# simonamtoft/downsampled-diffusion

Measured on AMD Instinct MI355X. Metric: images/sec (T=1000 sampling), 256x256 dDDPM-x3, higher is better.
Workload: dtype f32

## Files before the change

### downsampled-diffusion_amd/csrc/attention.hip

```cpp
#include <cstdlib>

#include "cluster_sync.h"
#include "conv_common.h"

namespace ddk {

constexpr int DH = 32;

constexpr int PART = DH + DH + DH * DH;

__global__ __launch_bounds__(256) void linattn_context_kernel(const float* __restrict__ qkv, float* __restrict__ ctx,
                                                              float* __restrict__ part, int HW, int heads, int splits, int rows_per_split,
                                                              int kv_only) {
    __shared__ __attribute__((aligned(16))) float stage[4 * 32 * 33];
    float* kexp = stage;
    float* vs = stage + 64 * DH;
    __shared__ float smax[8 * DH];
    const int bh = blockIdx.x / splits, sp = blockIdx.x % splits;
    const int b = bh / heads, h = bh % heads;
    const int HC = heads * DH, RS = (kv_only ? 2 : 3) * HC;
    const float* base = qkv + (long long)b * HW * RS;
    const float* kp = base + (kv_only ? 0 : HC) + h * DH;
    const float* vp = kp + HC;
    const int tid = threadIdx.x;
// ... 650 lines not shown
constexpr int AS_REC = 1152;
constexpr int AS_CNT = 32;
constexpr int AS_RING = 4;

template <int ROWS>
struct AttnSplitGeom {
    static_assert(ROWS == 128 || ROWS == 32, "half of a 16x16 or of an 8x8 map");
    static constexpr int XP = ROWS / 8;
    static constexpr int NP = XP + 12;
    static constexpr int SLOT = (ROWS + 96) * 32;
    static constexpr int NB = ROWS == 128 ? 3 : 1;
    static constexpr int UNITS = ROWS == 128 ? 4 : 3;
    static constexpr int KPART = UNITS * NB * 16 * 64;
    static constexpr int SCR = KPART > 8 * 32 * 33 ? KPART : 8 * 32 * 33;
    static constexpr int RING_FL = AS_RING * SLOT;
    static_assert(SCR + 2 * ROWS * DH + ROWS * (DH + 1) <= RING_FL, "k, v, q of the half live behind the scratch area in the drained ring");
    static constexpr int TAIL = DH * (DH + 4) + 2 * ROWS + 16 * DH + 16 * DH + DH + 192 + AS_REC + 32;
    static constexpr int LDS_FL = RING_FL + TAIL;
};

struct AttnSplitParams {
    const float* x;
    const float* w;
    const float* c1;
    const float* c2;
    float eps;
    float* ctx;
    float* out;
    unsigned* cnt;
    float* rec;
    unsigned* fail;
    int C;
};

__device__ __forceinline__ void wait_vmcnt_le(int n) {
    if (n >= 8) wait_vmcnt<8>();
    else if (n >= 6) wait_vmcnt<6>();
    else if (n >= 4) wait_vmcnt<4>();
    else if (n >= 3) wait_vmcnt<3>();
    else if (n >= 2) wait_vmcnt<2>();
    else wait_vmcnt<0>();
}

template <int ROWS>
__global__ __launch_bounds__(512) void attn_split_kernel(const AttnSplitParams p) {
    using G = AttnSplitGeom<ROWS>;
    constexpr int HW = 2 * ROWS, HC = 4 * DH;
    extern __shared__ __attribute__((aligned(16))) float smem[];
    float* scr = smem;
    float* ks = smem + G::SCR;
    float* vs = ks + ROWS * DH;
    float* qs = vs + ROWS * DH;
    float* cs = smem + G::RING_FL;
    float* rowstat = cs + DH * (DH + 4);
    float* smax = rowstat + 2 * ROWS;
    float* dpart = smax + 16 * DH;
    float* mx = dpart + 16 * DH;
    float* cfold = mx + DH;
    float* own = cfold + 192;
    int* gave_up = reinterpret_cast<int*>(own + AS_REC);
    const int tid = threadIdx.x, lane = tid & 63;
    const int wid = __builtin_amdgcn_readfirstlane(tid >> 6);
    const int half = blockIdx.x, h = blockIdx.y, b = blockIdx.z;
    const int C = p.C, nch = C >> 5;
    const float* xb = p.x + ((long long)b * HW + half * ROWS) * C;
    const unsigned lds_base = (unsigned)(size_t)(__attribute__((address_space(3))) float*)smem;

    const int prow = lane >> 3, ppos = lane & 7;
    const int npw = (G::NP - wid + 7) >> 3;
    unsigned voff[4];
#pragma unroll
    for (int j = 0; j < 4; ++j) {
        const int pj = wid + 8 * j;
        const int r = 8 * (pj < G::XP ? pj : pj - G::XP) + prow;
        const int src = pj < G::XP ? r : (r >> 5) * HC + h * DH + (r & 31);
        voff[j] = (unsigned)((src * C + ((ppos ^ ((r >> 1) & 7)) << 2)) * 4);
    }
    auto issue = [&](int chunk) {
        const unsigned dst = lds_base + (unsigned)(((chunk & (AS_RING - 1)) * G::SLOT) * 4);
#pragma unroll
        for (int j = 0; j < 4; ++j) {
            const int pj = wid + 8 * j;
            if (pj < G::NP) lds_dma16_s(pj < G::XP ? xb : p.w, voff[j] + (unsigned)(chunk * 128), dst + (unsigned)(pj * 1024));
        }
    };
    for (int c = 0; c < AS_RING - 1 && c < nch; ++c) issue(c);
    if (tid < 192) {
        const int n = tid % 96;
        const int col = (n >> 5) * HC + h * DH + (n & 31);
        cfold[tid] = tid < 96 ? p.c1[col] : p.c2[col];
    }
    if (tid < 4 * ROWS) {
        const int row = tid >> 2, sub = tid & 3, n16 = C >> 4;
        const float4* rp = reinterpret_cast<const float4*>(xb + (long long)row * C);
        float4 v[16];
        float s = 0.f;
#pragma unroll
        for (int i = 0; i < 16; ++i)
            if (i < n16) {
                v[i] = rp[sub + 4 * i];
                s += (v[i].x + v[i].y) + (v[i].z + v[i].w);
            }
        s += __shfl_xor(s, 1, 64);
        s += __shfl_xor(s, 2, 64);
        const float inv_c = 1.0f / (float)C;
        const float mean = s * inv_c;
        float qq = 0.f;
#pragma unroll
        for (int i = 0; i < 16; ++i)
            if (i < n16) {
                const float a0 = v[i].x - mean, a1 = v[i].y - mean, a2 = v[i].z - mean, a3 = v[i].w - mean;
                qq += (a0 * a0 + a1 * a1) + (a2 * a2 + a3 * a3);
            }
        qq += __shfl_xor(qq, 1, 64);
        qq += __shfl_xor(qq, 2, 64);
        if (sub == 0) {
            const float r = 1.0f / (sqrtf(qq * inv_c) + p.eps);
            rowstat[2 * row] = r;
            rowstat[2 * row + 1] = r * mean;
        }
    }

    const int pl = lane & 31, hl = lane >> 5;
    const bool active = ROWS == 128 || wid < 6;
    const int kh = ROWS == 128 ? wid >> 2 : (wid >= 3 ? 1 : 0);
    const int unit = ROWS == 128 ? (wid & 3) : (wid >= 3 ? wid - 3 : wid);
    const int pb = ROWS == 128 ? unit : 0, blk0 = ROWS == 128 ? 0 : unit;
    f32x16 acc[G::NB];
#pragma unroll
    for (int i = 0; i < G::NB; ++i)
#pragma unroll
        for (int r = 0; r < 16; ++r) acc[i][r] = 0.f;
    const int fsw = (pl >> 1) & 7;
    for (int c = 0; c < nch; ++c) {
        const int later = nch - 1 - c < AS_RING - 2 ? nch - 1 - c : AS_RING - 2;
        wait_vmcnt_le(later * npw);
        asm volatile("s_waitcnt lgkmcnt(0)\n\ts_barrier" ::: "memory");
        if (c + AS_RING - 1 < nch) issue(c + AS_RING - 1);
        if (active) {
            const float* Xs = smem + (c & (AS_RING - 1)) * G::SLOT + pb * (32 * 32);
            const float* Ws = smem + (c & (AS_RING - 1)) * G::SLOT + ROWS * 32 + blk0 * (32 * 32);
#pragma unroll
            for (int q2 = 0; q2 < 2; ++q2) {
                const int off = pl * 32 + (((2 * (2 * kh + q2) + hl) ^ fsw) << 2);
                const float4 xv = *reinterpret_cast<const float4*>(Xs + off);
                float4 wv[G::NB];
#pragma unroll
                for (int i = 0; i < G::NB; ++i) wv[i] = *reinterpret_cast<const float4*>(Ws + i * (32 * 32) + off);
#pragma unroll
                for (int e = 0; e < 4; ++e) {
                    const float xe = e == 0 ? xv.x : e == 1 ? xv.y : e == 2 ? xv.z : xv.w;
#pragma unroll
                    for (int i = 0; i < G::NB; ++i)
                        acc[i] = __builtin_amdgcn_mfma_f32_32x32x2f32(e == 0 ? wv[i].x : e == 1 ? wv[i].y : e == 2 ? wv[i].z : wv[i].w, xe, acc[i], 0, 0, 0);
                }
            }
        }
    }
    __syncthreads();
    if (active && kh == 1) {
#pragma unroll
        for (int i = 0; i < G::NB; ++i)
#pragma unroll
            for (int r = 0; r < 16; ++r) scr[((unit * G::NB + i) * 16 + r) * 64 + lane] = acc[i][r];
    }
    __syncthreads();
    if (active && kh == 0) {
        const int n = pb * 32 + pl;
        const float r = rowstat[2 * n], rm = rowstat[2 * n + 1];
#pragma unroll
        for (int i = 0; i < G::NB; ++i) {
            const int blk = blk0 + i;
#pragma unroll
            for (int q = 0; q < 4; ++q) {
                const int d0 = 8 * q + 4 * hl;
                float o4[4];
#pragma unroll
                for (int e = 0; e < 4; ++e) {
                    const float a = acc[i][4 * q + e] + scr[((unit * G::NB + i) * 16 + 4 * q + e) * 64 + lane];
                    o4[e] = r * a - rm * cfold[blk * 32 + d0 + e] + cfold[96 + blk * 32 + d0 + e];
                }
                if (blk == 0) {
#pragma unroll
                    for (int e = 0; e < 4; ++e) qs[n * (DH + 1) + d0 + e] = o4[e];
                } else {
                    *reinterpret_cast<float4*>((blk == 1 ? ks : vs) + n * DH + d0) = make_float4(o4[0], o4[1], o4[2], o4[3]);
                }
            }
        }
    }
    __syncthreads();

    {
        const int d = tid & 31, ng = tid >> 5;
        float m = -INFINITY;
        for (int n = ng; n < ROWS; n += 16) m = fmaxf(m, ks[n * DH + d]);
        smax[ng * DH + d] = m;
        __syncthreads();
        if (tid < DH) {
            float mm = smax[tid];
#pragma unroll
            for (int j = 1; j < 16; ++j) mm = fmaxf(mm, smax[j * DH + tid]);
            mx[tid] = mm;
        }
        __syncthreads();
// ... 31 lines not shown
#pragma unroll
            for (int w = 1; w < 8; ++w) t += scr[(w * 32 + md) * 33 + me0 + e];
            own[2 * DH + md * DH + me0 + e] = t;
        }
        if (me0 == 0) { own[md] = mx[md]; own[DH + md] = den; }
    }
    __syncthreads();
    unsigned* cnt = p.cnt + (b * 4 + h) * AS_CNT;
    float* rec = p.rec + (long long)(b * 4 + h) * 2 * AS_REC;
    if (wid == 0) {
        unsigned* mine = reinterpret_cast<unsigned*>(rec + half * AS_REC);
#pragma unroll
        for (int i = 0; i < (2 * DH + DH * DH) / 64; ++i)
            __hip_atomic_store(mine + lane + 64 * i, __float_as_uint(own[lane + 64 * i]), __ATOMIC_RELAXED, __HIP_MEMORY_SCOPE_AGENT);
        asm volatile("s_waitcnt vmcnt(0)" ::: "memory");
        if (lane == 0) {
            __hip_atomic_fetch_add(cnt, 1u, __ATOMIC_RELAXED, __HIP_MEMORY_SCOPE_AGENT);
            *gave_up = cl_wait_ge<2>(cnt, 2u, p.fail) ? 1 : 0;
        }
    }
    __syncthreads();
    const bool poisoned = *gave_up != 0;
    if (tid < 256) {
        const unsigned* theirs = reinterpret_cast<const unsigned*>(rec + (half ^ 1) * AS_REC);
        const float tm = __uint_as_float(__hip_atomic_load(theirs + md, __ATOMIC_RELAXED, __HIP_MEMORY_SCOPE_AGENT));
        const float td = __uint_as_float(__hip_atomic_load(theirs + DH + md, __ATOMIC_RELAXED, __HIP_MEMORY_SCOPE_AGENT));
        float ta[4];
#pragma unroll
        for (int e = 0; e < 4; ++e)
            ta[e] = __uint_as_float(__hip_atomic_load(theirs + 2 * DH + md * DH + me0 + e, __ATOMIC_RELAXED, __HIP_MEMORY_SCOPE_AGENT));
        if (tid == 0) cl_depart(cnt, cnt + 1, 2u);
        const float om = own[md], od = own[DH + md];
        const float m0 = half ? tm : om, m1 = half ? om : tm;
        const float d0 = half ? td : od, d1 = half ? od : td;
        const float M = fmaxf(m0, m1);
// ... 9 lines not shown
            const float a0 = half ? ta[e] : oa, a1 = half ? oa : ta[e];
            float a = 0.f;
            a += a0 * w0;
            a += a1 * w1;
            c4[e] = a * inv;
            cs[md * (DH + 4) + me0 + e] = c4[e];
        }
        if (half == 0) *reinterpret_cast<float4*>(p.ctx + (((long long)b * 4 + h) * DH + md) * DH + me0) = make_float4(c4[0], c4[1], c4[2], c4[3]);
    }
    __syncthreads();
    if (wid < ROWS / 32) {
        const int n0 = wid * 32;
        f32x16 oacc;
#pragma unroll
        for (int r = 0; r < 16; ++r) oacc[r] = 0.f;
        const float* qp = qs + (n0 + pl) * (DH + 1) + hl;
        const float* cp = cs + hl * (DH + 4) + pl;
#pragma unroll
        for (int j = 0; j < DH / 2; ++j) oacc = __builtin_amdgcn_mfma_f32_32x32x2f32(qp[2 * j], cp[2 * j * (DH + 4)], oacc, 0, 0, 0);
        float* op = p.out + ((long long)b * HW + half * ROWS + n0) * HC + h * DH + pl;
#pragma unroll
        for (int r = 0; r < 16; ++r) op[((r & 3) + 8 * (r >> 2) + 4 * hl) * HC] = oacc[r];
    }
}

__global__ __launch_bounds__(256) void qkv_operand_pack_kernel(const float* __restrict__ lnw, float* __restrict__ wop, int heads, int cp,
                                                               long long total) {
    const int nch = cp >> 5, HC = heads * DH;
    for (long long idx = blockIdx.x * 256LL + threadIdx.x; idx < total; idx += (long long)gridDim.x * 256) {
        const int j = (int)(idx & 3), lane = (int)((idx >> 2) & 63), half = (int)((idx >> 8) & 1);
        long long r = idx >> 9;
        const int nb = (int)(r % 6); r /= 6;
        const int chunk = (int)(r % nch);
        const int head = (int)(r / nch);
        const int o = (nb >> 1) * HC + head * DH + (nb & 1) * 16 + (lane & 15);
        const int i = chunk * 32 + (lane >> 4) * 8 + half * 4 + j;
        wop[idx] = lnw[(long long)o * cp + i];
    }
// ... 178 lines not shown
            const int n = nq * 32 + tid;
            a1[(long long)b * FOLD_C + n] = u1;
            a2[(long long)b * FOLD_C + n] = u2 + (bout ? bout[n] : 0.f);
        }
    }
}

int linattn_small_qkv_init_device() {
    DDK_HIP(hipFuncSetAttribute(reinterpret_cast<const void*>(attn_kvctx_kernel), hipFuncAttributeMaxDynamicSharedMemorySize,
                                (int)(KC_LDS_FLOATS * sizeof(float))));
    DDK_HIP(hipFuncSetAttribute(reinterpret_cast<const void*>(attn_fold_kernel), hipFuncAttributeMaxDynamicSharedMemorySize,
                                (int)(FOLD_LDS_FLOATS * sizeof(float))));
    DDK_HIP(hipFuncSetAttribute(reinterpret_cast<const void*>(linattn_small_kernel<256>), hipFuncAttributeMaxDynamicSharedMemorySize, 160 * 1024));
    DDK_HIP(hipFuncSetAttribute(reinterpret_cast<const void*>(linattn_small_qkv_kernel<1>), hipFuncAttributeMaxDynamicSharedMemorySize, 160 * 1024));
    DDK_HIP(hipFuncSetAttribute(reinterpret_cast<const void*>(linattn_small_qkv_kernel<4>), hipFuncAttributeMaxDynamicSharedMemorySize, 160 * 1024));
    DDK_HIP(hipFuncSetAttribute(reinterpret_cast<const void*>(attn_split_kernel<128>), hipFuncAttributeMaxDynamicSharedMemorySize,
                                (int)(AttnSplitGeom<128>::LDS_FL * sizeof(float))));
    DDK_HIP(hipFuncSetAttribute(reinterpret_cast<const void*>(attn_split_kernel<32>), hipFuncAttributeMaxDynamicSharedMemorySize,
                                (int)(AttnSplitGeom<32>::LDS_FL * sizeof(float))));
    return DDK_OK;
}

int qkv_operand_pack(const float* lnw, float* wop, int heads, int cp, hipStream_t st) {
    DDK_REQUIRE(lnw && wop && heads > 0 && cp > 0 && cp % 32 == 0, "qkv_operand_pack: arguments");
    const long long total = (long long)3 * heads * DH * cp;
    const long long blocks = ceil_div(total, 256);
    hipLaunchKernelGGL(qkv_operand_pack_kernel, dim3((unsigned)(blocks < 2048 ? blocks : 2048)), dim3(256), 0, st, lnw, wop, heads, cp, total);
    return check_launch("qkv_operand_pack_kernel");
}

int linattn_small_qkv(const float* x, const float* wop, const float* c1, const float* c2, float ln_eps, float* ctx, float* out, int B, int HW,
                      int C, int heads, hipStream_t st) {
// ... 37 lines not shown
    hipLaunchKernelGGL(linattn_merge_kernel, dim3(B * 4), dim3(256), 0, st, static_cast<const float*>(workspace), ctx, s);
    return check_launch("linattn_merge_kernel");
}

constexpr int AS_CUS = 256;
bool attn_split_ok(int B, int HW, int C, int heads) {
    return B > 0 && (HW == 64 || HW == 256) && C >= 32 && C <= 256 && C % 32 == 0 && heads == 4 && 8 * (long long)B <= AS_CUS &&
           conv_wino_cluster_device_ok();
}
size_t attn_split_counter_words(int B) { return (size_t)B * 4 * AS_CNT; }
size_t attn_split_record_floats(int B) { return (size_t)B * 4 * 2 * AS_REC; }
size_t attn_split_workspace_bytes(int B) { return B > 0 ? (32 + attn_split_counter_words(B) + attn_split_record_floats(B)) * sizeof(float) : 0; }
unsigned attention_cluster_timeouts() { return cl_timeouts_read(); }

int attn_split(const float* x, const float* w, const float* c1, const float* c2, float ln_eps, float* ctx, float* out, int B, int HW, int C,
               unsigned* counters, float* records, unsigned* fail, hipStream_t st) {
    DDK_REQUIRE(x && w && c1 && c2 && ctx && out && counters && records, "attn_split: null pointer");
    DDK_REQUIRE(attn_split_ok(B, HW, C, 4), "attn_split: needs H*W of 64 or 256, C % 32 == 0, C <= 256, 4 heads, 8 * B <= the CU count of a whole MI355X");
    DDK_REQUIRE(aligned16(x) && aligned16(w) && aligned16(ctx) && aligned16(out) && aligned16(counters) && aligned16(records), "attn_split: alignment");
    DDK_TRY(ensure_device_init());
    const AttnSplitParams p{x, w, c1, c2, ln_eps, ctx, out, counters, records, fail, C};
    if (HW == 256)
        hipLaunchKernelGGL(attn_split_kernel<128>, dim3(2, 4, (unsigned)B), dim3(512), AttnSplitGeom<128>::LDS_FL * sizeof(float), st, p);
    else
        hipLaunchKernelGGL(attn_split_kernel<32>, dim3(2, 4, (unsigned)B), dim3(512), AttnSplitGeom<32>::LDS_FL * sizeof(float), st, p);
    return check_launch("attn_split_kernel");
}

bool attn_fold_ok(int C, int heads) { return C == FOLD_C && heads * DH == FOLD_C; }
size_t attn_fold_out_floats(int B) { return (size_t)B * (FOLD_C * FOLD_C + 2 * FOLD_C); }

int attn_fold(const float* ctx, const float* wqg, const float* c1q, const float* c2q, const float* wout, const float* bout, float* A,
              float* a1, float* a2, int B, int C, int heads, hipStream_t st) {
    DDK_REQUIRE(ctx && wqg && c1q && c2q && wout && A && a1 && a2 && B > 0, "attn_fold: arguments");
    DDK_REQUIRE(attn_fold_ok(C, heads), "attn_fold: C == 128 and heads * 32 == 128 only");
    DDK_REQUIRE(aligned16(ctx) && aligned16(wout) && aligned16(A), "attn_fold: alignment");
    DDK_TRY(ensure_device_init());
// ... 19 lines not shown
    return ddk::linattn_context(qkv, ctx, B, HW, heads, workspace, workspace_bytes, ddk::as_stream(s), false);
}
int ddk_linattn_context_kv(const float* kv, float* ctx, int B, int HW, int heads, void* workspace, size_t workspace_bytes, ddk_stream_t s) {
    return ddk::linattn_context(kv, ctx, B, HW, heads, workspace, workspace_bytes, ddk::as_stream(s), true);
}
size_t ddk_attention_kv_context_workspace_bytes(int B, int HW) { return ddk::attn_kvctx_workspace_bytes(B, HW); }
int ddk_attention_kv_context_ok(int B, int HW, int C, int heads) { return ddk::attn_kvctx_ok(B, HW, C, heads) ? 1 : 0; }
int ddk_attention_kv_context(const float* x, const float* w_kv, const float* c1, const float* c2, float ln_eps, float* ctx, int B, int HW,
                             void* workspace, size_t workspace_bytes, ddk_stream_t s) {
    return ddk::attn_kvctx(x, w_kv, c1, c2, ln_eps, ctx, B, HW, workspace, workspace_bytes, ddk::as_stream(s));
}
size_t ddk_attention_split_workspace_bytes(int B) { return ddk::attn_split_workspace_bytes(B); }
int ddk_attention_split_ok(int B, int HW, int C, int heads) { return ddk::attn_split_ok(B, HW, C, heads) ? 1 : 0; }
int ddk_attention_split_from_x(const float* x, const float* w_folded, const float* c1, const float* c2, float ln_eps, float* ctx, float* out,
                               int B, int HW, int C, int heads, void* workspace, size_t workspace_bytes, ddk_stream_t s) {
    using namespace ddk;
    DDK_REQUIRE(workspace && B > 0 && heads == 4, "attention_split_from_x: arguments (4 heads)");
    if (workspace_bytes < attn_split_workspace_bytes(B)) {
        set_error("attention_split_from_x: workspace too small (%zu < %zu)", workspace_bytes, attn_split_workspace_bytes(B));
        return DDK_ERR_WORKSPACE;
    }
    unsigned* words = static_cast<unsigned*>(workspace);
    return attn_split(x, w_folded, c1, c2, ln_eps, ctx, out, B, HW, C, words + 32, static_cast<float*>(workspace) + 32 + attn_split_counter_words(B),
                      words, as_stream(s));
}
int ddk_attention_fold(const float* ctx, const float* wqg, const float* c1q, const float* c2q, const float* wout, const float* bout, float* A,
                       float* a1, float* a2, int B, int C, int heads, ddk_stream_t s) {
    return ddk::attn_fold(ctx, wqg, c1q, c2q, wout, bout, A, a1, a2, B, C, heads, ddk::as_stream(s));
}
int ddk_linattn_fused_small(const float* qkv, float* ctx, float* out, int B, int HW, int heads, ddk_stream_t s) {
    return ddk::linattn_fused_small(qkv, ctx, out, B, HW, heads, ddk::as_stream(s));
}
int ddk_pack_qkv_operand(const float* folded_w, float* dst, int heads, int c_pad, ddk_stream_t s) {
    return ddk::qkv_operand_pack(folded_w, dst, heads, c_pad, ddk::as_stream(s));
}
int ddk_linattn_small_from_x(const float* x, const float* w_operand, const float* c1, const float* c2, float ln_eps, float* ctx, float* out,
                             int B, int HW, int C, int heads, ddk_stream_t s) {
    return ddk::linattn_small_qkv(x, w_operand, c1, c2, ln_eps, ctx, out, B, HW, C, heads, ddk::as_stream(s));
}
int ddk_linattn_apply(const float* qkv, const float* ctx, float* out, int B, int HW, int heads, ddk_stream_t s) {
    return ddk::linattn_apply(qkv, ctx, out, B, HW, heads, ddk::as_stream(s));
}
}
```

### downsampled-diffusion_amd/csrc/ddk_internal.h

```cpp
#pragma once
#include <hip/hip_runtime.h>

#include <cstdarg>
#include <cstddef>
#include <cstdint>
#include <cstdio>

#include "ddk.h"

#ifdef DDK_HOST_SANITIZE
#include "host_sanitize.h"
#endif

namespace ddk {

void set_error(const char* fmt, ...);

inline int fail_arg(const char* what) {
    set_error("bad argument: %s", what);
    return DDK_ERR_ARG;
}

inline int check_launch(const char* what) {
    hipError_t e = hipGetLastError();
// ... 206 lines not shown
                    bool kv_only = false);
bool attn_fold_ok(int C, int heads);
bool attn_kvctx_ok(int B, int HW, int C, int heads);
size_t attn_kvctx_workspace_bytes(int B, int HW);
int attn_kvctx(const float* x, const float* w_kv, const float* c1, const float* c2, float ln_eps, float* ctx, int B, int HW, void* workspace,
               size_t workspace_bytes, hipStream_t st);
size_t attn_fold_out_floats(int B);
int attn_fold(const float* ctx, const float* wqg, const float* c1q, const float* c2q, const float* wout, const float* bout, float* A,
              float* a1, float* a2, int B, int C, int heads, hipStream_t st);
int linattn_apply(const float* qkv, const float* ctx, float* out, int B, int HW, int heads, hipStream_t st);
int linattn_fused_small(const float* qkv, float* ctx, float* out, int B, int HW, int heads, hipStream_t st);
bool attn_split_ok(int B, int HW, int C, int heads);
size_t attn_split_counter_words(int B);
size_t attn_split_record_floats(int B);
int attn_split(const float* x, const float* w, const float* c1, const float* c2, float ln_eps, float* ctx, float* out, int B, int HW, int C,
               unsigned* counters, float* records, unsigned* fail, hipStream_t st);
bool linattn_small_qkv_ok(int HW, int C);
int linattn_small_qkv_init_device();
int qkv_operand_pack(const float* lnw, float* wop, int heads, int cp, hipStream_t st);
int linattn_small_qkv(const float* x, const float* wop, const float* c1, const float* c2, float ln_eps, float* ctx, float* out, int B, int HW,
                      int C, int heads, hipStream_t st);
int time_mlp(const int64_t* t, const float* freqs, const float* w1t, const float* b1, const float* w2t, const float* b2,
             float* act, float* raw, int B, int dim, hipStream_t st);
int time_proj(const float* act, const float* wt, const float* bias, float* out, int B, int dim, int n_out, hipStream_t st);
int conv1x1_small_n(const float* x, const float* w, const float* bias, float* out, long long M, int C, int n_out, hipStream_t st);
struct InpaintOps {
    const float* known;
    const float* mask;
    const float *ka, *kb;
    const float *ja, *jb;
};
// ... 154 lines not shown
```

### downsampled-diffusion_amd/ddk/lib.py

```python
import ctypes as C
import os

import torch

_HERE = os.path.dirname(os.path.abspath(__file__))
LIB_PATH = os.environ.get("DDK_LIB", os.path.join(os.path.dirname(_HERE), "csrc", "libddk.so"))


class DDKError(RuntimeError):
    pass


ABI_VERSION = 400
ERR_CLUSTER = -4


class ConvArgs(C.Structure):
    _fields_ = [
        ("kind", C.c_int), ("src0", C.c_void_p), ("src1", C.c_void_p), ("c0", C.c_int), ("c1", C.c_int),
        ("weight", C.c_void_p), ("bias", C.c_void_p), ("resid", C.c_void_p), ("out", C.c_void_p),
        ("B", C.c_int), ("H", C.c_int), ("W", C.c_int), ("N", C.c_int), ("pre_mish", C.c_int), ("post_mish", C.c_int), ("defer_reduce", C.c_int),
        ("workspace", C.c_void_p), ("workspace_bytes", C.c_size_t), ("weight_wino", C.c_void_p),
        ("gn_partials", C.c_void_p), ("gn_groups", C.c_int), ("mish_out", C.c_void_p), ("dmish_src", C.c_void_p),
        ("skip_weight", C.c_void_p), ("skip_bias", C.c_void_p), ("skip_out", C.c_void_p), ("skip_slab_stride", C.c_longlong),
# ... 83 lines not shown
    "ddk_groupnorm_mish_partials_res1x1": (_I, [_P, _P, _I, _P, _P, _P, _I, _P, _P, _P, _I, _P, _I, _I, _I, _I, _F, _P]),
    "ddk_final_tail": (_I, [_P, _P, _I, _P, _P, _F, _P, _P, _I, _P, _P, _P, _P, _P, _P, _P, _P, _P, C.c_uint64, C.c_uint32, _I, _I, _I, _I, _P]),
    "ddk_pack_conv_weight_local": (_I, [_P, _P, _I, _I, _I, _P]),
    "ddk_pack_conv1x1_weight_local": (_I, [_P, _P, _I, _I, _I, _P]),
    "ddk_pack_convT_weight_local": (_I, [_P, _P, _I, _I, _P]),
    "ddk_pack_conv_weight_wino_local": (_I, [_P, _P, _I, _I, _I, _P]),
    "ddk_conv3x3_gn_mish_wino_ok": (_I, [_I, _I, _I, _I, _I, _I]),
    "ddk_conv3x3_gn_mish_wino": (_I, [_P, _I, _P, _I, _P, _P, _P, _P, _P, _I, _P, _P, _I, _I, _I, _I, _I, _F, _P]),
    "ddk_conv3x3_gn_mish_slabs": (_I, [_P, _I, _LL, _P, _I, _P, _P, _P, _P, _P, _I, _P, _I, _LL, _P, _P, _I, _I, _I, _I, _I, _F, _P]),
    "ddk_attention_kv_context_workspace_bytes": (_SZ, [_I, _I]),
    "ddk_attention_kv_context_ok": (_I, [_I, _I, _I, _I]),
    "ddk_attention_kv_context": (_I, [_P, _P, _P, _P, _F, _P, _I, _I, _P, _SZ, _P]),
    "ddk_attention_split_workspace_bytes": (_SZ, [_I]),
    "ddk_attention_split_ok": (_I, [_I, _I, _I, _I]),
    "ddk_attention_split_from_x": (_I, [_P, _P, _P, _P, _F, _P, _P, _I, _I, _I, _I, _P, _SZ, _P]),
    "ddk_pack_qkv_operand": (_I, [_P, _P, _I, _I, _P]),
    "ddk_linattn_small_from_x": (_I, [_P, _P, _P, _P, _F, _P, _P, _I, _I, _I, _I, _P]),
    "ddk_conv3x3_gn_mish_ok": (_I, [_I, _I, _I, _I, _I, _I]),
    "ddk_conv3x3_gn_mish": (_I, [_P, _I, _P, _I, _P, _P, _P, _P, _P, _I, _P, _P, _I, _I, _I, _I, _I, _F, _P]),
    "ddk_conv_workspace_bytes": (_SZ, [_I, _I, _I, _I, _I, _I]),
    "ddk_conv_splits": (_I, [_I, _I, _I, _I, _I, _I]),
    "ddk_conv_forward": (_I, [C.POINTER(ConvArgs), _P]),
    "ddk_debug_read_stamps": (_I, [_P]),
    "ddk_groupnorm_mish": (_I, [_P, _P, _P, _P, _I, _P, _P, _I, _I, _I, _I, _F, _P, _SZ, _P]),
    "ddk_groupnorm_workspace_bytes": (_SZ, [_I, _I, _I, _I]),
    "ddk_groupnorm_mish_slabs": (_I, [_P, _I, _LL, _P, _P, _P, _P, _I, _P, _P, _I, _I, _I, _I, _F, _P]),
    "ddk_chan_layernorm": (_I, [_P, _P, _P, _P, _LL, _I, _F, _P]),
    "ddk_mish": (_I, [_P, _P, _LL, _P]),
    "ddk_tanh": (_I, [_P, _P, _LL, _P]),
    "ddk_avgpool2": (_I, [_P, _P, _I, _I, _I, _I, _P]),
# ... 218 lines not shown
```

### downsampled-diffusion_amd/ddk/ops.py

```python
import ctypes as C
import math

import torch

from . import lib as L

CONV3X3_S1, CONV3X3_S2, CONV1X1, CONVT4X4_S2 = 0, 1, 2, 3
GN_GROUPS, GN_EPS, LN_EPS = 8, 1e-5, 1e-5


def pad32(c):
    return (c + 31) // 32 * 32


class _PackEntry:
    __slots__ = ("wref", "out", "job", "fresh", "pooled")


_pack_cache = {}
_weights_epoch = [0]
_pack_table = {}
pack_stats = {"single": 0, "batched_launches": 0, "batched_jobs": 0}
_graph_tables = []
_graph_keep = [_graph_tables]
# ... 1512 lines not shown
    wop = torch.empty_like(lnw)
    lib = L.load()
    L.check(lib.ddk_pack_qkv_operand(L.ptr(lnw), L.ptr(wop), heads, cp, L.stream()), "pack_qkv_operand")
    ctx = torch.empty((b, heads, 32, 32), device=x.device, dtype=torch.float32)
    out = torch.empty((b, h, w, heads * 32), device=x.device, dtype=torch.float32)
    L.check(lib.ddk_linattn_small_from_x(L.ptr(_f32(x)), L.ptr(wop), L.ptr(c1), L.ptr(c2), eps, L.ptr(ctx), L.ptr(out), b, h * w, c, heads,
                                         L.stream()), "linattn_small_from_x")
    return out, ctx


def attention_split_workspace(batch, device):
    nbytes = L.load().ddk_attention_split_workspace_bytes(batch)
    return torch.zeros(max(nbytes, 128) // 4, device=device, dtype=torch.float32)


def attention_split_from_x(x, w_qkv, ln_g, ln_b, heads=4, eps=LN_EPS, workspace=None):
    b, h, w, c = x.shape
    lib = L.load()
    if not lib.ddk_attention_split_ok(b, h * w, c, heads):
        raise L.DDKError(f"attention_split_from_x: shape {tuple(x.shape)} with {heads} heads not eligible "
                         "(H*W of 64 or 256, C % 32 == 0, C <= 256, 4 heads, 8 * B <= the CU count)")
    wq = w_qkv.reshape(w_qkv.shape[0], -1).to(torch.float32)
    g, bb = ln_g.reshape(-1).to(torch.float32), ln_b.reshape(-1).to(torch.float32)
    lnw = (wq * g[None, :]).contiguous()
    c1 = lnw.sum(dim=1).contiguous()
    c2 = (wq * bb[None, :]).sum(dim=1).contiguous()
    ws = attention_split_workspace(b, x.device) if workspace is None else workspace
    ctx = torch.empty((b, heads, 32, 32), device=x.device, dtype=torch.float32)
    out = torch.empty((b, h, w, heads * 32), device=x.device, dtype=torch.float32)
    L.check(lib.ddk_attention_split_from_x(L.ptr(_f32(x)), L.ptr(lnw), L.ptr(c1), L.ptr(c2), eps, L.ptr(ctx), L.ptr(out), b, h * w, c, heads,
                                           L.ptr(ws), ws.numel() * 4, L.stream()), "attention_split_from_x")
    return out, ctx


def linattn_train(qkv, heads=4):
    out, ctx = linattn(qkv, heads)
    b, h, w, _ = qkv.shape
    stats = torch.empty((b, heads, 2, 32), device=qkv.device, dtype=torch.float32)
    lib = L.load()
    nbytes = lib.ddk_linattn_train_workspace_bytes(b, h * w, heads)
    ws = _ws(qkv.device, nbytes, "linattn_train") if nbytes else None
    L.check(lib.ddk_linattn_stats(L.ptr(qkv), L.ptr(stats), b, h * w, heads, L.ptr(ws), nbytes, L.stream()), "linattn_stats")
    return out, ctx, stats


def linattn_bwd(qkv, dout, ctx, stats, heads=4):
# ... 317 lines not shown
```

### include/ddk.h

```cpp
#ifndef DDK_H
#define DDK_H

#include <stddef.h>
#include <stdint.h>

#ifdef __cplusplus
extern "C" {
#endif

typedef void* ddk_stream_t;

#define DDK_OK 0
#define DDK_ERR_ARG (-1)
#define DDK_ERR_HIP (-2)
#define DDK_ERR_WORKSPACE (-3)
#define DDK_ERR_CLUSTER (-4)

int ddk_version(void);
const char* ddk_last_error(void);
int ddk_device_ok(void);

int ddk_nchw_to_nhwc(const float* src, float* dst, int B, int C, int H, int W, int c_pad, ddk_stream_t s);
int ddk_nhwc_to_nchw(const float* src, float* dst, int B, int C, int H, int W, int c_stride, ddk_stream_t s);
int ddk_pad_channels(const float* src, float* dst, long long M, int C, int c_pad, ddk_stream_t s);
// ... 109 lines not shown
int ddk_add(const float* a, const float* b, float* out, long long n, ddk_stream_t s);

size_t ddk_linattn_context_workspace_bytes(int B, int HW, int heads);
int ddk_linattn_context(const float* qkv, float* ctx, int B, int HW, int heads, void* workspace, size_t workspace_bytes, ddk_stream_t s);
int ddk_linattn_context_kv(const float* kv, float* ctx, int B, int HW, int heads, void* workspace, size_t workspace_bytes, ddk_stream_t s);
int ddk_attention_fold(const float* ctx, const float* wqg, const float* c1q, const float* c2q, const float* wout, const float* bout, float* A,
                       float* a1, float* a2, int B, int C, int heads, ddk_stream_t s);
size_t ddk_attention_kv_context_workspace_bytes(int B, int HW);
int ddk_attention_kv_context_ok(int B, int HW, int C, int heads);
int ddk_attention_kv_context(const float* x, const float* w_kv, const float* c1, const float* c2, float ln_eps, float* ctx, int B, int HW,
                             void* workspace, size_t workspace_bytes, ddk_stream_t s);
size_t ddk_attention_split_workspace_bytes(int B);
int ddk_attention_split_ok(int B, int HW, int C, int heads);
int ddk_attention_split_from_x(const float* x, const float* w_folded, const float* c1, const float* c2, float ln_eps, float* ctx, float* out,
                               int B, int HW, int C, int heads, void* workspace, size_t workspace_bytes, ddk_stream_t s);
int ddk_linattn_fused_small(const float* qkv, float* ctx, float* out, int B, int HW, int heads, ddk_stream_t s);
int ddk_linattn_apply(const float* qkv, const float* ctx, float* out, int B, int HW, int heads, ddk_stream_t s);
int ddk_pack_qkv_operand(const float* folded_w, float* dst, int heads, int c_pad, ddk_stream_t s);
int ddk_linattn_small_from_x(const float* x, const float* w_operand, const float* c1, const float* c2, float ln_eps, float* ctx,
                             float* out, int B, int HW, int C, int heads, ddk_stream_t s);

int ddk_time_mlp(const int64_t* t, const float* freqs, const float* w1t, const float* b1, const float* w2t,
                 const float* b2, float* act, float* raw, int B, int dim, ddk_stream_t s);
int ddk_time_proj(const float* act, const float* wt, const float* bias, float* out, int B, int dim, int n_out,
                  ddk_stream_t s);

int ddk_conv1x1_small_n(const float* x, const float* w, const float* bias, float* out, long long M, int C,
                        int n_out, ddk_stream_t s);

int ddk_q_sample(const float* x, const float* eps, const int64_t* t, const float* sqrt_acp,
// ... 372 lines not shown
```

Before: 27.05.

## Unroll attention split chunk loop at compile time and defer q-fold past cluster publish

Adds compile-time chunk-count specialisations of the split attention kernel for C=128 and C=256. These fully unroll the DMA ring loop with constant waitcnt values, immediate LDS offsets and scheduling barriers, and issue the next DMA after the MFMA block. The q-third of the fold is moved after the cross-block publish, with its own LDS parking area, so that work overlaps the wait for the partner half, and q values are preloaded into registers before that wait. The LayerNorm stats loop is also made branch-free. The cost is larger LDS use, more code size, and optional tuning timestamp instrumentation.

```diff
diff --git a/downsampled-diffusion_amd/csrc/attention.hip b/downsampled-diffusion_amd/csrc/attention.hip
--- a/downsampled-diffusion_amd/csrc/attention.hip
+++ b/downsampled-diffusion_amd/csrc/attention.hip
@@ -1,4 +1,6 @@
 #include <cstdlib>
+#include <type_traits>
+#include <utility>
 
 #include "cluster_sync.h"
 #include "conv_common.h"
@@ -688,9 +690,13 @@
     static constexpr int KPART = UNITS * NB * 16 * 64;
     static constexpr int SCR = KPART > 8 * 32 * 33 ? KPART : 8 * 32 * 33;
     static constexpr int RING_FL = AS_RING * SLOT;
-    static_assert(SCR + 2 * ROWS * DH + ROWS * (DH + 1) <= RING_FL, "k, v, q of the half live behind the scratch area in the drained ring");
+    static constexpr int QPART = SCR + 2 * ROWS * DH + ROWS * (DH + 1);
+    static constexpr int QUNITS = ROWS == 128 ? 4 : 1;
+    static constexpr int BODY_FL = QPART + QUNITS * 16 * 64 > RING_FL ? QPART + QUNITS * 16 * 64 : RING_FL;
     static constexpr int TAIL = DH * (DH + 4) + 2 * ROWS + 16 * DH + 16 * DH + DH + 192 + AS_REC + 32;
-    static constexpr int LDS_FL = RING_FL + TAIL;
+    static constexpr int LDS_FL = BODY_FL + TAIL;
+    static constexpr int FRAG_IMM_MAX = (SLOT + (NB - 1) * 32 * 32) * 4;
+    static_assert(FRAG_IMM_MAX < 65536, "the DS instruction's 16-bit offset field");
 };
 
 struct AttnSplitParams {
@@ -716,16 +722,31 @@
     else wait_vmcnt<0>();
 }
 
-template <int ROWS>
+template <class F, int... I>
+__device__ __forceinline__ void static_chunks(F&& f, std::integer_sequence<int, I...>) { (f(std::integral_constant<int, I>{}), ...); }
+
+#ifdef DDK_TUNING
+__device__ unsigned long long g_as_stamps[8 * 256];
+#define AS_STAMP(x) do { asm volatile("s_memtime %0\n\ts_waitcnt lgkmcnt(0)" : "=s"(x) :: "memory"); } while (0)
+#else
+#define AS_STAMP(x) do { } while (0)
+#endif
+
+template <int ROWS, int NCH = 0>
 __global__ __launch_bounds__(512) void attn_split_kernel(const AttnSplitParams p) {
     using G = AttnSplitGeom<ROWS>;
+    static_assert(NCH == 0 || (ROWS == 128 && NCH >= AS_RING - 1 && NCH <= 8), "unrolled chunk loop: the 16x16 sites only");
     constexpr int HW = 2 * ROWS, HC = 4 * DH;
     extern __shared__ __attribute__((aligned(16))) float smem[];
+    unsigned long long st_entry = 0, st_loop0 = 0, st_loop1 = 0, st_pub = 0, st_met = 0;
+    (void)st_entry; (void)st_loop0; (void)st_loop1; (void)st_pub; (void)st_met;
+    AS_STAMP(st_entry);
     float* scr = smem;
     float* ks = smem + G::SCR;
     float* vs = ks + ROWS * DH;
     float* qs = vs + ROWS * DH;
-    float* cs = smem + G::RING_FL;
+    float* qpart = smem + G::QPART;
+    float* cs = smem + G::BODY_FL;
     float* rowstat = cs + DH * (DH + 4);
     float* smax = rowstat + 2 * ROWS;
     float* dpart = smax + 16 * DH;
@@ -736,7 +757,7 @@
     const int tid = threadIdx.x, lane = tid & 63;
     const int wid = __builtin_amdgcn_readfirstlane(tid >> 6);
     const int half = blockIdx.x, h = blockIdx.y, b = blockIdx.z;
-    const int C = p.C, nch = C >> 5;
+    const int C = NCH ? NCH * 32 : p.C, nch = C >> 5;
     const float* xb = p.x + ((long long)b * HW + half * ROWS) * C;
     const unsigned lds_base = (unsigned)(size_t)(__attribute__((address_space(3))) float*)smem;
 
@@ -750,12 +771,18 @@
         const int src = pj < G::XP ? r : (r >> 5) * HC + h * DH + (r & 31);
         voff[j] = (unsigned)((src * C + ((ppos ^ ((r >> 1) & 7)) << 2)) * 4);
     }
-    auto issue = [&](int chunk) {
+    auto issue = [&](auto chunk) {
         const unsigned dst = lds_base + (unsigned)(((chunk & (AS_RING - 1)) * G::SLOT) * 4);
 #pragma unroll
         for (int j = 0; j < 4; ++j) {
             const int pj = wid + 8 * j;
-            if (pj < G::NP) lds_dma16_s(pj < G::XP ? xb : p.w, voff[j] + (unsigned)(chunk * 128), dst + (unsigned)(pj * 1024));
+            if constexpr (std::is_same<decltype(chunk), int>::value) {
+                if (pj < G::NP) lds_dma16_s(pj < G::XP ? xb : p.w, voff[j] + (unsigned)(chunk * 128), dst + (unsigned)(pj * 1024));
+            } else {
+                static_assert(G::XP % 8 == 0, "a wave's piece j is x for every wave or for none");
+                if (8 * j + 7 < G::NP || pj < G::NP)
+                    lds_dma16_s((8 * j < G::XP ? xb : p.w) + decltype(chunk)::value * 32, voff[j], dst + (unsigned)(pj * 1024));
+            }
         }
     };
     for (int c = 0; c < AS_RING - 1 && c < nch; ++c) issue(c);
@@ -768,24 +795,26 @@
         const int row = tid >> 2, sub = tid & 3, n16 = C >> 4;
         const float4* rp = reinterpret_cast<const float4*>(xb + (long long)row * C);
         float4 v[16];
+#pragma unroll
+        for (int i = 0; i < 16; ++i) v[i] = rp[sub + 4 * (i < n16 ? i : n16 - 1)];
         float s = 0.f;
 #pragma unroll
-        for (int i = 0; i < 16; ++i)
-            if (i < n16) {
-                v[i] = rp[sub + 4 * i];
-                s += (v[i].x + v[i].y) + (v[i].z + v[i].w);
-            }
+        for (int i = 0; i < 16; ++i) {
+            const float t = s + ((v[i].x + v[i].y) + (v[i].z + v[i].w));
+            s = i < n16 ? t : s;
+        }
         s += __shfl_xor(s, 1, 64);
         s += __shfl_xor(s, 2, 64);
         const float inv_c = 1.0f / (float)C;
-        const float mean = s * inv_c;
+        float mean = s * inv_c;
+        asm volatile("" : "+v"(mean));
         float qq = 0.f;
 #pragma unroll
-        for (int i = 0; i < 16; ++i)
-            if (i < n16) {
-                const float a0 = v[i].x - mean, a1 = v[i].y - mean, a2 = v[i].z - mean, a3 = v[i].w - mean;
-                qq += (a0 * a0 + a1 * a1) + (a2 * a2 + a3 * a3);
-            }
+        for (int i = 0; i < 16; ++i) {
+            const float a0 = v[i].x - mean, a1 = v[i].y - mean, a2 = v[i].z - mean, a3 = v[i].w - mean;
+            const float t = qq + ((a0 * a0 + a1 * a1) + (a2 * a2 + a3 * a3));
+            qq = i < n16 ? t : qq;
+        }
         qq += __shfl_xor(qq, 1, 64);
         qq += __shfl_xor(qq, 2, 64);
         if (sub == 0) {
@@ -806,63 +835,130 @@
 #pragma unroll
         for (int r = 0; r < 16; ++r) acc[i][r] = 0.f;
     const int fsw = (pl >> 1) & 7;
-    for (int c = 0; c < nch; ++c) {
-        const int later = nch - 1 - c < AS_RING - 2 ? nch - 1 - c : AS_RING - 2;
-        wait_vmcnt_le(later * npw);
+    int foff[2];
+#pragma unroll
+    for (int q2 = 0; q2 < 2; ++q2) foff[q2] = pl * 32 + (((2 * (2 * kh + q2) + hl) ^ fsw) << 2);
+    const float *fx[2][2], *fw[2][2];
+#pragma unroll
+    for (int rh = 0; rh < 2; ++rh)
+#pragma unroll
+        for (int q2 = 0; q2 < 2; ++q2) {
+            fx[rh][q2] = smem + 2 * rh * G::SLOT + pb * (32 * 32) + foff[q2];
+            fw[rh][q2] = smem + 2 * rh * G::SLOT + ROWS * 32 + blk0 * (32 * 32) + foff[q2];
+        }
+    auto chunk_step = [&](auto chunk) {
+        constexpr bool RT = std::is_same<decltype(chunk), int>::value;
+        const int c = chunk, slot = c & (AS_RING - 1);
+        if constexpr (RT) {
+            const int later = nch - 1 - c < AS_RING - 2 ? nch - 1 - c : AS_RING - 2;
+            wait_vmcnt_le(later * npw);
+        } else {
+            constexpr int LATER = NCH - 1 - decltype(chunk)::value < AS_RING - 2 ? NCH - 1 - decltype(chunk)::value : AS_RING - 2;
+            if (npw == 4) wait_vmcnt<4 * LATER>();
+            else wait_vmcnt<3 * LATER>();
+        }
         asm volatile("s_waitcnt lgkmcnt(0)\n\ts_barrier" ::: "memory");
-        if (c + AS_RING - 1 < nch) issue(c + AS_RING - 1);
+        if constexpr (RT) {
+            if (c + AS_RING - 1 < nch) issue(c + AS_RING - 1);
+        }
+#if defined(DDK_TUNING) && defined(DDK_AS_DMA_FIRST)
+        if constexpr (!RT) {
+            if constexpr (decltype(chunk)::value + AS_RING - 1 < NCH) issue(std::integral_constant<int, decltype(chunk)::value + AS_RING - 1>{});
+        }
+#endif
         if (active) {
-            const float* Xs = smem + (c & (AS_RING - 1)) * G::SLOT + pb * (32 * 32);
-            const float* Ws = smem + (c & (AS_RING - 1)) * G::SLOT + ROWS * 32 + blk0 * (32 * 32);
+            float4 xv[2], wv[2][G::NB];
 #pragma unroll
             for (int q2 = 0; q2 < 2; ++q2) {
-                const int off = pl * 32 + (((2 * (2 * kh + q2) + hl) ^ fsw) << 2);
-                const float4 xv = *reinterpret_cast<const float4*>(Xs + off);
-                float4 wv[G::NB];
-#pragma unroll
-                for (int i = 0; i < G::NB; ++i) wv[i] = *reinterpret_cast<const float4*>(Ws + i * (32 * 32) + off);
+                const float *Xs, *Ws;
+                if constexpr (RT) {
+                    Xs = smem + slot * G::SLOT + pb * (32 * 32) + foff[q2];
+                    Ws = smem + slot * G::SLOT + ROWS * 32 + blk0 * (32 * 32) + foff[q2];
+                } else {
+                    constexpr int S = decltype(chunk)::value & (AS_RING - 1);
+                    Xs = fx[S >> 1][q2] + (S & 1) * G::SLOT;
+                    Ws = fw[S >> 1][q2] + (S & 1) * G::SLOT;
+                }
+                xv[q2] = *reinterpret_cast<const float4*>(Xs);
+#pragma unroll
+                for (int i = 0; i < G::NB; ++i) wv[q2][i] = *reinterpret_cast<const float4*>(Ws + i * (32 * 32));
+            }
+            if constexpr (!RT) __builtin_amdgcn_sched_barrier(0);
+#if defined(DDK_TUNING) && defined(DDK_AS_PRIO)
+            if constexpr (!RT) __builtin_amdgcn_s_setprio(DDK_AS_PRIO);
+#endif
+#pragma unroll
+            for (int q2 = 0; q2 < 2; ++q2)
 #pragma unroll
                 for (int e = 0; e < 4; ++e) {
-                    const float xe = e == 0 ? xv.x : e == 1 ? xv.y : e == 2 ? xv.z : xv.w;
+                    const float xe = e == 0 ? xv[q2].x : e == 1 ? xv[q2].y : e == 2 ? xv[q2].z : xv[q2].w;
 #pragma unroll
                     for (int i = 0; i < G::NB; ++i)
-                        acc[i] = __builtin_amdgcn_mfma_f32_32x32x2f32(e == 0 ? wv[i].x : e == 1 ? wv[i].y : e == 2 ? wv[i].z : wv[i].w, xe, acc[i], 0, 0, 0);
+                        acc[i] = __builtin_amdgcn_mfma_f32_32x32x2f32(e == 0 ? wv[q2][i].x : e == 1 ? wv[q2][i].y : e == 2 ? wv[q2][i].z : wv[q2][i].w, xe,
+                                                                      acc[i], 0, 0, 0);
+                }
+#if defined(DDK_TUNING) && defined(DDK_AS_PRIO)
+            if constexpr (!RT) __builtin_amdgcn_s_setprio(0);
+#endif
+            if constexpr (!RT) __builtin_amdgcn_sched_barrier(0);
+        }
+#if !defined(DDK_TUNING) || !defined(DDK_AS_DMA_FIRST)
+        if constexpr (!RT) {
+            if constexpr (decltype(chunk)::value + AS_RING - 1 < NCH) issue(std::integral_constant<int, decltype(chunk)::value + AS_RING - 1>{});
+        }
+#endif
+    };
+    AS_STAMP(st_loop0);
+    if constexpr (NCH == 0) {
+        for (int c = 0; c < nch; ++c) chunk_step(c);
+    } else {
+        static_chunks(chunk_step, std::make_integer_sequence<int, NCH>{});
+    }
+    AS_STAMP(st_loop1);
+    __syncthreads();
+    auto park_upper = [&](bool q_third) {
+        if (active && kh == 1) {
+#pragma unroll
+            for (int i = 0; i < G::NB; ++i) {
+                if ((blk0 + i == 0) != q_third) continue;
+                float* dst = blk0 + i == 0 ? qpart + (ROWS == 128 ? unit : 0) * (16 * 64) : scr + (unit * G::NB + i) * (16 * 64);
+#pragma unroll
+                for (int r = 0; r < 16; ++r) dst[r * 64 + lane] = acc[i][r];
+            }
+        }
+    };
+    auto meet_and_fold = [&](bool q_third) {
+        if (active && kh == 0) {
+            const int n = pb * 32 + pl;
+            const float r = rowstat[2 * n], rm = rowstat[2 * n + 1];
+#pragma unroll
+            for (int i = 0; i < G::NB; ++i) {
+                const int blk = blk0 + i;
+                if ((blk == 0) != q_third) continue;
+                const float* up = blk == 0 ? qpart + (ROWS == 128 ? unit : 0) * (16 * 64) : scr + (unit * G::NB + i) * (16 * 64);
+#pragma unroll
+                for (int q = 0; q < 4; ++q) {
+                    const int d0 = 8 * q + 4 * hl;
+                    float o4[4];
+#pragma unroll
+                    for (int e = 0; e < 4; ++e) {
+                        const float a = acc[i][4 * q + e] + up[(4 * q + e) * 64 + lane];
+                        o4[e] = r * a - rm * cfold[blk * 32 + d0 + e] + cfold[96 + blk * 32 + d0 + e];
+                    }
+                    if (blk == 0) {
+#pragma unroll
+                        for (int e = 0; e < 4; ++e) qs[n * (DH + 1) + d0 + e] = o4[e];
+                    } else {
+                        *reinterpret_cast<float4*>((blk == 1 ? ks : vs) + n * DH + d0) = make_float4(o4[0], o4[1], o4[2], o4[3]);
+                    }
                 }
             }
         }
-    }
-    __syncthreads();
-    if (active && kh == 1) {
-#pragma unroll
-        for (int i = 0; i < G::NB; ++i)
-#pragma unroll
-            for (int r = 0; r < 16; ++r) scr[((unit * G::NB + i) * 16 + r) * 64 + lane] = acc[i][r];
-    }
-    __syncthreads();
-    if (active && kh == 0) {
-        const int n = pb * 32 + pl;
-        const float r = rowstat[2 * n], rm = rowstat[2 * n + 1];
-#pragma unroll
-        for (int i = 0; i < G::NB; ++i) {
-            const int blk = blk0 + i;
-#pragma unroll
-            for (int q = 0; q < 4; ++q) {
-                const int d0 = 8 * q + 4 * hl;
-                float o4[4];
-#pragma unroll
-                for (int e = 0; e < 4; ++e) {
-                    const float a = acc[i][4 * q + e] + scr[((unit * G::NB + i) * 16 + 4 * q + e) * 64 + lane];
-                    o4[e] = r * a - rm * cfold[blk * 32 + d0 + e] + cfold[96 + blk * 32 + d0 + e];
-                }
-                if (blk == 0) {
-#pragma unroll
-                    for (int e = 0; e < 4; ++e) qs[n * (DH + 1) + d0 + e] = o4[e];
-                } else {
-                    *reinterpret_cast<float4*>((blk == 1 ? ks : vs) + n * DH + d0) = make_float4(o4[0], o4[1], o4[2], o4[3]);
-                }
-            }
-        }
-    }
+    };
+    park_upper(false);
+    park_upper(true);
+    __syncthreads();
+    meet_and_fold(false);
     __syncthreads();
 
     {
@@ -924,11 +1020,21 @@
         for (int i = 0; i < (2 * DH + DH * DH) / 64; ++i)
             __hip_atomic_store(mine + lane + 64 * i, __float_as_uint(own[lane + 64 * i]), __ATOMIC_RELAXED, __HIP_MEMORY_SCOPE_AGENT);
         asm volatile("s_waitcnt vmcnt(0)" ::: "memory");
-        if (lane == 0) {
-            __hip_atomic_fetch_add(cnt, 1u, __ATOMIC_RELAXED, __HIP_MEMORY_SCOPE_AGENT);
-            *gave_up = cl_wait_ge<2>(cnt, 2u, p.fail) ? 1 : 0;
-        }
-    }
+        if (lane == 0) __hip_atomic_fetch_add(cnt, 1u, __ATOMIC_RELAXED, __HIP_MEMORY_SCOPE_AGENT);
+    }
+    AS_STAMP(st_pub);
+    meet_and_fold(true);
+    float qv[DH / 2];
+    if (wid < ROWS / 32) {
+        __builtin_amdgcn_fence(__ATOMIC_RELEASE, "wavefront");
+        __builtin_amdgcn_wave_barrier();
+        __builtin_amdgcn_fence(__ATOMIC_ACQUIRE, "wavefront");
+        const float* qp = qs + (wid * 32 + pl) * (DH + 1) + hl;
+#pragma unroll
+        for (int j = 0; j < DH / 2; ++j) qv[j] = qp[2 * j];
+    }
+    if (tid == 0) *gave_up = cl_wait_ge<2>(cnt, 2u, p.fail) ? 1 : 0;
+    AS_STAMP(st_met);
     __syncthreads();
     const bool poisoned = *gave_up != 0;
     if (tid < 256) {
@@ -968,14 +1074,22 @@
         f32x16 oacc;
 #pragma unroll
         for (int r = 0; r < 16; ++r) oacc[r] = 0.f;
-        const float* qp = qs + (n0 + pl) * (DH + 1) + hl;
         const float* cp = cs + hl * (DH + 4) + pl;
 #pragma unroll
-        for (int j = 0; j < DH / 2; ++j) oacc = __builtin_amdgcn_mfma_f32_32x32x2f32(qp[2 * j], cp[2 * j * (DH + 4)], oacc, 0, 0, 0);
+        for (int j = 0; j < DH / 2; ++j) oacc = __builtin_amdgcn_mfma_f32_32x32x2f32(qv[j], cp[2 * j * (DH + 4)], oacc, 0, 0, 0);
         float* op = p.out + ((long long)b * HW + half * ROWS + n0) * HC + h * DH + pl;
 #pragma unroll
         for (int r = 0; r < 16; ++r) op[((r & 3) + 8 * (r >> 2) + 4 * hl) * HC] = oacc[r];
     }
+#ifdef DDK_TUNING
+    if (tid == 0) {
+        asm volatile("s_waitcnt vmcnt(0)" ::: "memory");
+        unsigned long long st_end;
+        AS_STAMP(st_end);
+        unsigned long long* o = g_as_stamps + ((blockIdx.z * 4 + blockIdx.y) * 2 + blockIdx.x) % 256 * 8;
+        o[0] = st_entry; o[1] = st_loop0; o[2] = st_loop1; o[3] = st_pub; o[4] = st_met; o[5] = st_end; o[6] = (unsigned long long)nch; o[7] = NCH ? 2 : 1;
+    }
+#endif
 }
 
 __global__ __launch_bounds__(256) void qkv_operand_pack_kernel(const float* __restrict__ lnw, float* __restrict__ wop, int heads, int cp,
@@ -1184,8 +1298,9 @@
     DDK_HIP(hipFuncSetAttribute(reinterpret_cast<const void*>(linattn_small_kernel<256>), hipFuncAttributeMaxDynamicSharedMemorySize, 160 * 1024));
     DDK_HIP(hipFuncSetAttribute(reinterpret_cast<const void*>(linattn_small_qkv_kernel<1>), hipFuncAttributeMaxDynamicSharedMemorySize, 160 * 1024));
     DDK_HIP(hipFuncSetAttribute(reinterpret_cast<const void*>(linattn_small_qkv_kernel<4>), hipFuncAttributeMaxDynamicSharedMemorySize, 160 * 1024));
-    DDK_HIP(hipFuncSetAttribute(reinterpret_cast<const void*>(attn_split_kernel<128>), hipFuncAttributeMaxDynamicSharedMemorySize,
-                                (int)(AttnSplitGeom<128>::LDS_FL * sizeof(float))));
+    for (const void* k : {reinterpret_cast<const void*>(attn_split_kernel<128>), reinterpret_cast<const void*>(attn_split_kernel<128, 4>),
+                          reinterpret_cast<const void*>(attn_split_kernel<128, 8>)})
+        DDK_HIP(hipFuncSetAttribute(k, hipFuncAttributeMaxDynamicSharedMemorySize, (int)(AttnSplitGeom<128>::LDS_FL * sizeof(float))));
     DDK_HIP(hipFuncSetAttribute(reinterpret_cast<const void*>(attn_split_kernel<32>), hipFuncAttributeMaxDynamicSharedMemorySize,
                                 (int)(AttnSplitGeom<32>::LDS_FL * sizeof(float))));
     return DDK_OK;
@@ -1253,13 +1368,17 @@
 unsigned attention_cluster_timeouts() { return cl_timeouts_read(); }
 
 int attn_split(const float* x, const float* w, const float* c1, const float* c2, float ln_eps, float* ctx, float* out, int B, int HW, int C,
-               unsigned* counters, float* records, unsigned* fail, hipStream_t st) {
+               unsigned* counters, float* records, unsigned* fail, hipStream_t st, bool runtime_loop) {
     DDK_REQUIRE(x && w && c1 && c2 && ctx && out && counters && records, "attn_split: null pointer");
     DDK_REQUIRE(attn_split_ok(B, HW, C, 4), "attn_split: needs H*W of 64 or 256, C % 32 == 0, C <= 256, 4 heads, 8 * B <= the CU count of a whole MI355X");
     DDK_REQUIRE(aligned16(x) && aligned16(w) && aligned16(ctx) && aligned16(out) && aligned16(counters) && aligned16(records), "attn_split: alignment");
     DDK_TRY(ensure_device_init());
     const AttnSplitParams p{x, w, c1, c2, ln_eps, ctx, out, counters, records, fail, C};
-    if (HW == 256)
+    if (HW == 256 && C == 256 && !runtime_loop)
+        hipLaunchKernelGGL((attn_split_kernel<128, 8>), dim3(2, 4, (unsigned)B), dim3(512), AttnSplitGeom<128>::LDS_FL * sizeof(float), st, p);
+    else if (HW == 256 && C == 128 && !runtime_loop)
+        hipLaunchKernelGGL((attn_split_kernel<128, 4>), dim3(2, 4, (unsigned)B), dim3(512), AttnSplitGeom<128>::LDS_FL * sizeof(float), st, p);
+    else if (HW == 256)
         hipLaunchKernelGGL(attn_split_kernel<128>, dim3(2, 4, (unsigned)B), dim3(512), AttnSplitGeom<128>::LDS_FL * sizeof(float), st, p);
     else
         hipLaunchKernelGGL(attn_split_kernel<32>, dim3(2, 4, (unsigned)B), dim3(512), AttnSplitGeom<32>::LDS_FL * sizeof(float), st, p);
@@ -1309,7 +1428,12 @@
 int ddk_attention_split_ok(int B, int HW, int C, int heads) { return ddk::attn_split_ok(B, HW, C, heads) ? 1 : 0; }
 int ddk_attention_split_from_x(const float* x, const float* w_folded, const float* c1, const float* c2, float ln_eps, float* ctx, float* out,
                                int B, int HW, int C, int heads, void* workspace, size_t workspace_bytes, ddk_stream_t s) {
+    return ddk_attention_split_from_x_form(x, w_folded, c1, c2, ln_eps, ctx, out, B, HW, C, heads, workspace, workspace_bytes, 0, s);
+}
+int ddk_attention_split_from_x_form(const float* x, const float* w_folded, const float* c1, const float* c2, float ln_eps, float* ctx, float* out,
+                                    int B, int HW, int C, int heads, void* workspace, size_t workspace_bytes, int loop_form, ddk_stream_t s) {
     using namespace ddk;
+    DDK_REQUIRE(loop_form == 0 || loop_form == 1, "attention_split_from_x: loop_form is 0 (as dispatched) or 1 (run-time chunk loop)");
     DDK_REQUIRE(workspace && B > 0 && heads == 4, "attention_split_from_x: arguments (4 heads)");
     if (workspace_bytes < attn_split_workspace_bytes(B)) {
         set_error("attention_split_from_x: workspace too small (%zu < %zu)", workspace_bytes, attn_split_workspace_bytes(B));
@@ -1317,7 +1441,7 @@
     }
     unsigned* words = static_cast<unsigned*>(workspace);
     return attn_split(x, w_folded, c1, c2, ln_eps, ctx, out, B, HW, C, words + 32, static_cast<float*>(workspace) + 32 + attn_split_counter_words(B),
-                      words, as_stream(s));
+                      words, as_stream(s), loop_form == 1);
 }
 int ddk_attention_fold(const float* ctx, const float* wqg, const float* c1q, const float* c2q, const float* wout, const float* bout, float* A,
                        float* a1, float* a2, int B, int C, int heads, ddk_stream_t s) {
@@ -1337,3 +1461,12 @@
     return ddk::linattn_apply(qkv, ctx, out, B, HW, heads, ddk::as_stream(s));
 }
 }
+
+#ifdef DDK_TUNING
+extern "C" int ddk_debug_read_attn_split_stamps(unsigned long long* host_out) {
+    if (hipDeviceSynchronize() != hipSuccess) return -2;
+    if (hipMemcpyFromSymbol(host_out, HIP_SYMBOL(ddk::g_as_stamps), sizeof(unsigned long long) * 8 * 256) != hipSuccess) return -2;
+    static unsigned long long zeros[8 * 256];
+    return hipMemcpyToSymbol(HIP_SYMBOL(ddk::g_as_stamps), zeros, sizeof(zeros)) == hipSuccess ? 0 : -2;
+}
+#endif
diff --git a/downsampled-diffusion_amd/csrc/ddk_internal.h b/downsampled-diffusion_amd/csrc/ddk_internal.h
--- a/downsampled-diffusion_amd/csrc/ddk_internal.h
+++ b/downsampled-diffusion_amd/csrc/ddk_internal.h
@@ -244,7 +244,7 @@
 size_t attn_split_counter_words(int B);
 size_t attn_split_record_floats(int B);
 int attn_split(const float* x, const float* w, const float* c1, const float* c2, float ln_eps, float* ctx, float* out, int B, int HW, int C,
-               unsigned* counters, float* records, unsigned* fail, hipStream_t st);
+               unsigned* counters, float* records, unsigned* fail, hipStream_t st, bool runtime_loop = false);
 bool linattn_small_qkv_ok(int HW, int C);
 int linattn_small_qkv_init_device();
 int qkv_operand_pack(const float* lnw, float* wop, int heads, int cp, hipStream_t st);
diff --git a/downsampled-diffusion_amd/ddk/lib.py b/downsampled-diffusion_amd/ddk/lib.py
--- a/downsampled-diffusion_amd/ddk/lib.py
+++ b/downsampled-diffusion_amd/ddk/lib.py
@@ -121,6 +121,7 @@
     "ddk_attention_split_workspace_bytes": (_SZ, [_I]),
     "ddk_attention_split_ok": (_I, [_I, _I, _I, _I]),
     "ddk_attention_split_from_x": (_I, [_P, _P, _P, _P, _F, _P, _P, _I, _I, _I, _I, _P, _SZ, _P]),
+    "ddk_attention_split_from_x_form": (_I, [_P, _P, _P, _P, _F, _P, _P, _I, _I, _I, _I, _P, _SZ, _I, _P]),
     "ddk_pack_qkv_operand": (_I, [_P, _P, _I, _I, _P]),
     "ddk_linattn_small_from_x": (_I, [_P, _P, _P, _P, _F, _P, _P, _I, _I, _I, _I, _P]),
     "ddk_conv3x3_gn_mish_ok": (_I, [_I, _I, _I, _I, _I, _I]),
diff --git a/downsampled-diffusion_amd/ddk/ops.py b/downsampled-diffusion_amd/ddk/ops.py
--- a/downsampled-diffusion_amd/ddk/ops.py
+++ b/downsampled-diffusion_amd/ddk/ops.py
@@ -1550,7 +1550,7 @@
     return torch.zeros(max(nbytes, 128) // 4, device=device, dtype=torch.float32)
 
 
-def attention_split_from_x(x, w_qkv, ln_g, ln_b, heads=4, eps=LN_EPS, workspace=None):
+def attention_split_from_x(x, w_qkv, ln_g, ln_b, heads=4, eps=LN_EPS, workspace=None, loop_form=0):
     b, h, w, c = x.shape
     lib = L.load()
     if not lib.ddk_attention_split_ok(b, h * w, c, heads):
@@ -1564,8 +1564,8 @@
     ws = attention_split_workspace(b, x.device) if workspace is None else workspace
     ctx = torch.empty((b, heads, 32, 32), device=x.device, dtype=torch.float32)
     out = torch.empty((b, h, w, heads * 32), device=x.device, dtype=torch.float32)
-    L.check(lib.ddk_attention_split_from_x(L.ptr(_f32(x)), L.ptr(lnw), L.ptr(c1), L.ptr(c2), eps, L.ptr(ctx), L.ptr(out), b, h * w, c, heads,
-                                           L.ptr(ws), ws.numel() * 4, L.stream()), "attention_split_from_x")
+    L.check(lib.ddk_attention_split_from_x_form(L.ptr(_f32(x)), L.ptr(lnw), L.ptr(c1), L.ptr(c2), eps, L.ptr(ctx), L.ptr(out), b, h * w, c,
+                                                heads, L.ptr(ws), ws.numel() * 4, loop_form, L.stream()), "attention_split_from_x")
     return out, ctx
 
 
diff --git a/include/ddk.h b/include/ddk.h
--- a/include/ddk.h
+++ b/include/ddk.h
@@ -147,6 +147,9 @@
 int ddk_attention_split_ok(int B, int HW, int C, int heads);
 int ddk_attention_split_from_x(const float* x, const float* w_folded, const float* c1, const float* c2, float ln_eps, float* ctx, float* out,
                                int B, int HW, int C, int heads, void* workspace, size_t workspace_bytes, ddk_stream_t s);
+int ddk_attention_split_from_x_form(const float* x, const float* w_folded, const float* c1, const float* c2, float ln_eps, float* ctx,
+                                    float* out, int B, int HW, int C, int heads, void* workspace, size_t workspace_bytes, int loop_form,
+                                    ddk_stream_t s);
 int ddk_linattn_fused_small(const float* qkv, float* ctx, float* out, int B, int HW, int heads, ddk_stream_t s);
 int ddk_linattn_apply(const float* qkv, const float* ctx, float* out, int B, int HW, int heads, ddk_stream_t s);
 int ddk_pack_qkv_operand(const float* folded_w, float* dst, int heads, int c_pad, ddk_stream_t s);
```

New measurement: 27.30 (median of 6 runs). No clear change (+0.9%).
